# titanium-47/decision-pretrained-transformer

Measured on NVIDIA B200. Metric: env-steps/sec (bandit rollout collect, H=500 dim=5), higher is better.
Workload: dtype f32

## Files before the change

decision-pretrained-transformer_b200/csrc/api.cu:

```cuda
#include "common.cuh"

namespace dpt {

static thread_local char g_err[512] = "";

void set_error(const char* fmt, ...) {
  va_list ap;
  va_start(ap, fmt);
  vsnprintf(g_err, sizeof(g_err), fmt, ap);
  va_end(ap);
}

int sm_count() {
  static thread_local int cached_dev = -1, cached = 0;
  int dev = 0;
  if (cudaGetDevice(&dev) != cudaSuccess) return 148;
  if (dev != cached_dev) {
    int n = 0;
    if (cudaDeviceGetAttribute(&n, cudaDevAttrMultiProcessorCount, dev) != cudaSuccess || n <= 0) n = 148;
    cached = n;
    cached_dev = dev;
  }
  return cached;
}

int pick_envs_per_cta(int N, int slots, int min_e, int max_e) {
  if (min_e < 1) min_e = 1;
  if (max_e < min_e) max_e = min_e;
  if (slots < 1) slots = 1;
  int best = -1;
  double best_eff = -1.0;
  for (int e = max_e; e >= min_e; --e) {
    const long grid = ((long)N + e - 1) / e;
    const long waves = (grid + slots - 1) / slots;
    if (waves < 3 && e > min_e) continue;
    const double eff = (double)grid / (double)(waves * slots);
    if (eff > best_eff + 1e-9) best_eff = eff, best = e;
  }
  return best < 0 ? min_e : best;
}

}

extern "C" int dpt_version(void) { return DPT_ABI_VERSION; }

extern "C" const char* dpt_last_error(void) { return dpt::g_err; }

extern "C" int dpt_device_info(int* sm_count, int* cc_major, int* cc_minor) {
  int dev = 0;
  DPT_CUDA(cudaGetDevice(&dev));
  int n = 0, maj = 0, min = 0;
  DPT_CUDA(cudaDeviceGetAttribute(&n, cudaDevAttrMultiProcessorCount, dev));
  DPT_CUDA(cudaDeviceGetAttribute(&maj, cudaDevAttrComputeCapabilityMajor, dev));
  DPT_CUDA(cudaDeviceGetAttribute(&min, cudaDevAttrComputeCapabilityMinor, dev));
  if (sm_count) *sm_count = n;
  if (cc_major) *cc_major = maj;
  if (cc_minor) *cc_minor = min;
  return DPT_OK;
}
```

decision-pretrained-transformer_b200/csrc/bandit_rollin.cu:

```cuda
#include <string.h>

#include <unordered_map>

#include "common.cuh"
#include "philox.cuh"

namespace dpt {

constexpr int RB_THREADS = 256;
constexpr int RB_WARPS = RB_THREADS / 32;
constexpr int RB_MAX_ENVS = 32;
constexpr int RB_MAX_D = 32;

enum { MODE_PHILOX = 0, MODE_PHILOX_DUMP = 1, MODE_INJECT = 2 };

struct RollinParams {
  const float* means;
  float var;
  int rtype;
  Key key;
  uint64_t env_id0;
  int N, H, d, envs_per_cta;
  float *ctx_s, *ctx_a, *ctx_ns, *ctx_r;
  uint8_t* acts_u8;
  double* stats;
  dpt_bandit_inject_t in;
  dpt_bandit_dump_t out;
};

__constant__ double c_cov_grid[11] = {0.0, .1, .2, .3, .4, .5, .6, .7, .8, .9, 1.0};

template <int MODE>
struct Thr {
  using type = uint32_t;
};
template <>
struct Thr<MODE_INJECT> {
  using type = double;
};

template <int MODE, int DMAX>
__device__ __forceinline__ void rollin_setup_env(const RollinParams& p, int env, int D, float* s_means,
                                                 typename Thr<MODE>::type* s_thr) {
  const uint64_t gid = p.env_id0 + (uint64_t)env;
  for (int j = 0; j < D; ++j) s_means[j] = p.means[(size_t)env * D + j];
  if (MODE == MODE_INJECT && p.in.actions != nullptr) return;
  int cov_idx, ridx;
  double probs[DMAX];
  if (MODE == MODE_INJECT) {
    cov_idx = p.in.cov_idx[env];
    ridx = p.in.rand_idx[env];
#pragma unroll
    for (int j = 0; j < DMAX; ++j)
      if (j < D) probs[j] = p.in.dir_probs[(size_t)env * D + j];
  } else {
    const uint4 w = philox_words(p.key, gid, 0, STREAM_ROLLIN_SETUP);
    cov_idx = (int)bounded(w.x, 11);
    ridx = (int)bounded(w.y, (uint32_t)D);
    double sum = 0.0;
#pragma unroll
    for (int b = 0; b < (DMAX + 3) / 4; ++b) {
      if (4 * b < D) {
        const uint4 g = philox_words(p.key, gid, 1 + b, STREAM_ROLLIN_SETUP);
#pragma unroll
        for (int i = 0; i < 4; ++i) {
          const int j = 4 * b + i;
          if (j < DMAX && j < D) {
            probs[j] = (double)(-__logf(u32_open0(word_of(g, i))));
            sum += probs[j];
          }
        }
      }
    }
// ... 29 lines not shown
      }
    }
  }
}

__device__ __forceinline__ void reduce_stats(const RollinParams& p, float sr, float sr2, float nopt) {
  double* stats = p.stats;
  __shared__ float s_part[3][RB_WARPS];
  const int lane = threadIdx.x & 31, warp = threadIdx.x >> 5;
#pragma unroll
  for (int o = 16; o > 0; o >>= 1) {
    sr += __shfl_xor_sync(0xffffffffu, sr, o);
    sr2 += __shfl_xor_sync(0xffffffffu, sr2, o);
    nopt += __shfl_xor_sync(0xffffffffu, nopt, o);
  }
  if (lane == 0) s_part[0][warp] = sr, s_part[1][warp] = sr2, s_part[2][warp] = nopt;
  __syncthreads();
  if (threadIdx.x < 3) {
    double acc = 0.0;
    for (int w = 0; w < RB_WARPS; ++w) acc += (double)s_part[threadIdx.x][w];
    atomicAdd(stats + threadIdx.x, acc);
  }
}

struct PeerPublish {
  double* dst[DPT_MAX_PEERS];
  int n;
};
__global__ void peer_publish_kernel(const double* __restrict__ stats, const PeerPublish pp) {
  const int r = threadIdx.x / 3, t = threadIdx.x - 3 * r;
  if (r < pp.n) asm volatile("st.global.relaxed.sys.f64 [%0], %1;" ::"l"(pp.dst[r] + t), "d"(stats[t]) : "memory");
}

__device__ __forceinline__ float2 add2(float2 a, float2 b) {
  float2 r;
  asm("add.rn.f32x2 %0, %1, %2;" : "=l"(reinterpret_cast<uint64_t&>(r)) : "l"(reinterpret_cast<uint64_t&>(a)), "l"(reinterpret_cast<uint64_t&>(b)));
  return r;
}
__device__ __forceinline__ float2 fma2(float2 a, float2 b, float2 c) {
  float2 r;
  asm("fma.rn.f32x2 %0, %1, %2, %3;"
      : "=l"(reinterpret_cast<uint64_t&>(r))
      : "l"(reinterpret_cast<uint64_t&>(a)), "l"(reinterpret_cast<uint64_t&>(b)), "l"(reinterpret_cast<uint64_t&>(c)));
  return r;
}

__device__ __forceinline__ int argmax_first(const float* m, int D) {
  int best = 0;
  for (int j = 1; j < D; ++j)
    if (m[j] > m[best]) best = j;
  return best;
}

template <int D, int MODE, int RT>
__global__ void __launch_bounds__(RB_THREADS) bandit_rollin_fast(const RollinParams p) {
  using thr_t = typename Thr<MODE>::type;
  __shared__ float s_means[RB_MAX_ENVS][D];
  __shared__ thr_t s_thr[RB_MAX_ENVS][D];
  __shared__ uint32_t s_optmask[RB_MAX_ENVS];
  const int tid = threadIdx.x, lane = tid & 31, warp = tid >> 5;
  const int env0 = blockIdx.x * p.envs_per_cta;
  const int ne = min(p.envs_per_cta, p.N - env0);
  const int H = p.H;

  if (warp == 0) {
    if (lane < ne) {
      rollin_setup_env<MODE, D>(p, env0 + lane, D, s_means[lane], s_thr[lane]);
      const int oa = argmax_first(s_means[lane], D);
      s_optmask[lane] = (1u << oa) | (1u << (D + oa));
    }
  } else {
    const size_t b = (size_t)env0 * H, e = (size_t)(env0 + ne) * H;
    fill_range(p.ctx_s, b, e, 1.0f, tid - 32, RB_THREADS - 32);
    fill_range(p.ctx_ns, b, e, 1.0f, tid - 32, RB_THREADS - 32);
  }
  __syncthreads();

  const int chunks = (H + 63) >> 6;
  const bool inj_actions = (MODE == MODE_INJECT) && p.in.actions != nullptr;
  float2 st_r = make_float2(0.f, 0.f), st_r2 = make_float2(0.f, 0.f);
  int st_opt = 0;
  const int de = RB_WARPS / chunks, dc = RB_WARPS - de * chunks;
  int e = warp / chunks, c = warp - e * chunks;
  for (; e < ne; e += de, c += dc) {
    if (c >= chunks) {
      c -= chunks, ++e;
      if (e >= ne) break;
    }
    const int env = env0 + e;
    const int h0 = c * 64 + 2 * lane;
    const size_t row = (size_t)env * H + h0;
    int a0 = 0, a1 = 0;
    float z0 = 0.f, z1 = 0.f;
    if (MODE != MODE_INJECT) {
      const uint4 w = philox_words(p.key, p.env_id0 + (uint64_t)env, (uint32_t)(c * 32 + lane), STREAM_ROLLIN_STEP);
      const uint32_t k0 = w.x >> 1, k1 = w.y >> 1;
#pragma unroll
      for (int j = 0; j < D - 1; ++j) {
        const uint32_t t = s_thr[e][j];
        a0 += (k0 >= t);
        a1 += (k1 >= t);
      }
      if (RT == DPT_REWARD_GAUSSIAN)
        box_muller(w.z, w.w, z0, z1);
      else
        z0 = u24(w.z), z1 = u24(w.w);
      if (MODE == MODE_PHILOX_DUMP && h0 < H) {
        if (p.out.u) {
          p.out.u[row] = (double)k0 * 4.656612873077392578125e-10;
          p.out.u[row + 1] = (double)k1 * 4.656612873077392578125e-10;
        }
        if (p.out.z) p.out.z[row] = z0, p.out.z[row + 1] = z1;
        if (p.out.actions) p.out.actions[row] = a0, p.out.actions[row + 1] = a1;
      }
    } else if (h0 < H) {
      if (inj_actions) {
        a0 = p.in.actions[row];
        a1 = p.in.actions[row + 1];
      } else {
        const double u0 = p.in.u[row], u1 = p.in.u[row + 1];
#pragma unroll
        for (int j = 0; j < D - 1; ++j) {
          const double t = s_thr[e][j];
          a0 += (t <= u0);
          a1 += (t <= u1);
        }
      }
      z0 = p.in.z[row];
      z1 = p.in.z[row + 1];
    }
    {
      const float m0 = s_means[e][a0], m1 = s_means[e][a1];
      const bool gauss = RT == DPT_REWARD_GAUSSIAN;
      const float r0 = gauss ? fmaf(p.var, z0, m0) : (z0 < m0 ? 1.f : 0.f);
      const float r1 = gauss ? fmaf(p.var, z1, m1) : (z1 < m1 ? 1.f : 0.f);
      st_stream_if(h0 < H, reinterpret_cast<float2*>(p.ctx_r + row), make_float2(r0, r1));
      if (p.stats && h0 < H) {
        const float2 rr = make_float2(r0, r1);
        st_r = add2(st_r, rr);
        st_r2 = fma2(rr, rr, st_r2);
      }
    }
    const uint32_t m = (1u << a0) | (1u << (D + a1));
    if (p.stats && h0 < H) st_opt += __popc(m & s_optmask[e]);
    float4* abase = reinterpret_cast<float4*>(p.ctx_a + ((size_t)env * H + (size_t)c * 64) * D);
    const int n_valid4 = (min(64, H - c * 64) * D) >> 2;
#pragma unroll
    for (int it = 0; it < (16 * D + 31) / 32; ++it) {
      const int q = it * 32 + lane;
      const int e0 = 4 * q;
      const int l0 = e0 / (2 * D);
      const int off = e0 - l0 * (2 * D);
      const uint32_t mlo = __shfl_sync(0xffffffffu, m, l0 & 31);
      const uint32_t mhi = __shfl_sync(0xffffffffu, m, (l0 + 1) & 31);
      const uint32_t bits = (uint32_t)(((((uint64_t)mhi) << (2 * D)) | mlo) >> off);
      const float4 v = make_float4((bits & 1u) ? 1.f : 0.f, (bits & 2u) ? 1.f : 0.f, (bits & 4u) ? 1.f : 0.f,
                                   (bits & 8u) ? 1.f : 0.f);
      st_stream_if(q < n_valid4, abase + q, v);
    }
  }
  if (p.stats) reduce_stats(p, st_r.x + st_r.y, st_r2.x + st_r2.y, (float)st_opt);
}

template <int MODE>
__global__ void __launch_bounds__(RB_THREADS) bandit_rollin_generic(const RollinParams p) {
  using thr_t = typename Thr<MODE>::type;
  __shared__ float s_means[RB_MAX_ENVS][RB_MAX_D];
  __shared__ thr_t s_thr[RB_MAX_ENVS][RB_MAX_D];
  __shared__ int s_opt[RB_MAX_ENVS];
  const int tid = threadIdx.x, lane = tid & 31, warp = tid >> 5;
  const int env0 = blockIdx.x * p.envs_per_cta;
  const int ne = min(p.envs_per_cta, p.N - env0);
  const int H = p.H, D = p.d;

  if (tid < ne) {
    rollin_setup_env<MODE, RB_MAX_D>(p, env0 + tid, D, s_means[tid], s_thr[tid]);
    s_opt[tid] = argmax_first(s_means[tid], D);
  }
  if (!p.acts_u8) {
    for (size_t i = (size_t)env0 * H + tid; i < (size_t)(env0 + ne) * H; i += RB_THREADS) {
      st_stream(p.ctx_s + i, 1.0f);
      st_stream(p.ctx_ns + i, 1.0f);
    }
  }
  __syncthreads();

  const int chunks = (H + 31) >> 5;
  const bool inj_actions = (MODE == MODE_INJECT) && p.in.actions != nullptr;
  float st_r = 0.f, st_r2 = 0.f, st_opt = 0.f;
  for (int task = warp; task < ne * chunks; task += RB_WARPS) {
    const int e = task / chunks, c = task - e * chunks;
    const int env = env0 + e;
    const int h = c * 32 + lane;
    const size_t row = (size_t)env * H + h;
    int a = 0;
    float z = 0.f;
    if (MODE != MODE_INJECT) {
      const uint4 w = philox_words(p.key, p.env_id0 + (uint64_t)env, (uint32_t)(h >> 1), STREAM_ROLLIN_STEP);
      const uint32_t k = ((h & 1) ? w.y : w.x) >> 1;
      for (int j = 0; j < D - 1; ++j) a += (k >= s_thr[e][j]);
      if (p.rtype == DPT_REWARD_GAUSSIAN) {
        float z0, z1;
        box_muller(w.z, w.w, z0, z1);
        z = (h & 1) ? z1 : z0;
      } else {
        z = u24((h & 1) ? w.w : w.z);
      }
      if (MODE == MODE_PHILOX_DUMP && h < H) {
        if (p.out.u) p.out.u[row] = (double)k * 4.656612873077392578125e-10;
        if (p.out.z) p.out.z[row] = z;
        if (p.out.actions) p.out.actions[row] = a;
      }
    } else if (h < H) {
      if (inj_actions) {
        a = p.in.actions[row];
      } else {
        const double u = p.in.u[row];
        for (int j = 0; j < D - 1; ++j) a += (s_thr[e][j] <= u);
      }
      z = p.in.z[row];
    }
    if (h < H) {
      const float ma = s_means[e][a];
      const float r = p.rtype == DPT_REWARD_GAUSSIAN ? fmaf(p.var, z, ma) : (z < ma ? 1.f : 0.f);
      st_stream(p.ctx_r + row, r);
      if (p.stats) st_r += r, st_r2 = fmaf(r, r, st_r2), st_opt += (float)(a == s_opt[e]);
    }
    if (p.acts_u8) {
      if (h < H) p.acts_u8[row] = (uint8_t)a;
      continue;
    }
    const int nvalid = min(32, H - c * 32) * D;
    float* abase = p.ctx_a + ((size_t)env * H + (size_t)c * 32) * D;
    for (int it = 0; it < D; ++it) {
      const int i = it * 32 + lane;
      const int s = i / D;
      const int as = __shfl_sync(0xffffffffu, a, s & 31);
      if (i < nvalid) st_stream(abase + i, (i - s * D) == as ? 1.f : 0.f);
    }
  }
  if (p.stats) reduce_stats(p, st_r, st_r2, st_opt);
}

template <typename K>
static int resident_ctas(K kern) {
  static thread_local std::unordered_map<const void*, int> cache;
  const void* key = reinterpret_cast<const void*>(kern);
  auto it = cache.find(key);
  if (it != cache.end()) return it->second;
  int n = 0;
  if (cudaOccupancyMaxActiveBlocksPerMultiprocessor(&n, kern, RB_THREADS, 0) != cudaSuccess || n < 1) n = 4;
  cache[key] = n;
  return n;
}

template <int MODE>
static void launch_mode(RollinParams p, bool fast, cudaStream_t st) {
  auto go = [&](auto kern) {
    const int per_sm = resident_ctas(kern);
    p.envs_per_cta = pick_envs_per_cta(p.N, sm_count() * per_sm, 1, RB_MAX_ENVS);
    const int grid = (p.N + p.envs_per_cta - 1) / p.envs_per_cta;
    kern<<<grid, RB_THREADS, 0, st>>>(p);
  };
  if (fast) {
    switch (p.d) {
#define DPT_CASE(DD)                                                   \
  case DD:                                                             \
    if (p.rtype == DPT_REWARD_GAUSSIAN)                                \
      go(bandit_rollin_fast<DD, MODE, DPT_REWARD_GAUSSIAN>);           \
    else                                                               \
      go(bandit_rollin_fast<DD, MODE, DPT_REWARD_BERNOULLI>);          \
    return;
      DPT_CASE(2)
      DPT_CASE(3)
      DPT_CASE(4)
      DPT_CASE(5)
      DPT_CASE(6)
      DPT_CASE(8)
      DPT_CASE(10)
      DPT_CASE(16)
#undef DPT_CASE
      default:
        break;
    }
  }
  go(bandit_rollin_generic<MODE>);
}

}

using namespace dpt;

static int bandit_rollin_impl(const float* means, float var, int reward_type, uint64_t seed, uint64_t env_id0, int N, int H, int d,
                              float* ctx_states, float* ctx_actions, float* ctx_next_states, float* ctx_rewards,
                              double* return_stats, const dpt_bandit_inject_t* inject, const dpt_bandit_dump_t* dump,
                              double* const* peer_dst, int n_peers, unsigned int* done_counter, void* stream,
                              uint8_t* acts_u8 = nullptr) {
  DPT_CHECK_ARG(N >= 0 && H >= 0, "dpt_bandit_rollin: N=%d H=%d must be >= 0", N, H);
  DPT_CHECK_ARG(reward_type == DPT_REWARD_GAUSSIAN || reward_type == DPT_REWARD_BERNOULLI,
                "dpt_bandit_rollin: unknown reward_type %d (0 uniform/gaussian, 1 bernoulli)", reward_type);
  DPT_CHECK_ARG(d >= 1 && d <= RB_MAX_D, "dpt_bandit_rollin: d=%d outside [1,%d]", d, RB_MAX_D);
  if (N == 0 || H == 0) return DPT_OK;
  DPT_CHECK_ARG(means && ctx_rewards && (acts_u8 || (ctx_states && ctx_actions && ctx_next_states)),
                "dpt_bandit_rollin: null means/context pointer");
  RollinParams p{};
  p.acts_u8 = acts_u8;
  p.means = means;
  p.var = var;
  p.rtype = reward_type;
  p.key = Key{(uint32_t)seed, (uint32_t)(seed >> 32)};
  p.env_id0 = env_id0;
  p.N = N, p.H = H, p.d = d;
  p.ctx_s = ctx_states, p.ctx_a = ctx_actions, p.ctx_ns = ctx_next_states, p.ctx_r = ctx_rewards;
  p.stats = return_stats;
  if (n_peers > 0)
    DPT_CHECK_ARG(n_peers <= DPT_MAX_PEERS && peer_dst && return_stats,
                  "dpt_bandit_rollin_p2p: needs return_stats and 1..%d peer pointers", DPT_MAX_PEERS);
  int mode = MODE_PHILOX;
  if (inject) {
    DPT_CHECK_ARG(!dump, "dpt_bandit_rollin: inject and dump are mutually exclusive");
    DPT_CHECK_ARG(inject->z, "dpt_bandit_rollin: inject->z is required");
    DPT_CHECK_ARG(inject->actions || (inject->cov_idx && inject->dir_probs && inject->rand_idx && inject->u),
                  "dpt_bandit_rollin: inject needs actions or (cov_idx, dir_probs, rand_idx, u)");
    p.in = *inject;
    mode = MODE_INJECT;
  } else if (dump) {
    p.out = *dump;
    mode = MODE_PHILOX_DUMP;
  }
  const bool fast = !acts_u8 && (H % 4 == 0) && 2 * d <= 32 && aligned16(ctx_states) && aligned16(ctx_actions) &&
                    aligned16(ctx_next_states) && aligned16(ctx_rewards);
  cudaStream_t st = (cudaStream_t)stream;
  if (mode == MODE_PHILOX)
    launch_mode<MODE_PHILOX>(p, fast, st);
  else if (mode == MODE_PHILOX_DUMP)
    launch_mode<MODE_PHILOX_DUMP>(p, fast, st);
  else
    launch_mode<MODE_INJECT>(p, fast, st);
  DPT_LAUNCH_CHECK();
  if (n_peers > 0) {
    PeerPublish pp{};
    for (int r = 0; r < n_peers; ++r) pp.dst[r] = peer_dst[r];
    pp.n = n_peers;
    peer_publish_kernel<<<1, 3 * DPT_MAX_PEERS <= 32 ? 32 : 3 * DPT_MAX_PEERS, 0, st>>>(return_stats, pp);
    DPT_LAUNCH_CHECK();
  }
  (void)done_counter;
  return DPT_OK;
}

extern "C" int dpt_bandit_rollin(const float* means, float var, int reward_type, uint64_t seed, uint64_t env_id0, int N, int H, int d,
                                 float* ctx_states, float* ctx_actions, float* ctx_next_states, float* ctx_rewards,
                                 double* return_stats, const dpt_bandit_inject_t* inject,
                                 const dpt_bandit_dump_t* dump, void* stream) {
  return bandit_rollin_impl(means, var, reward_type, seed, env_id0, N, H, d, ctx_states, ctx_actions, ctx_next_states,
                            ctx_rewards, return_stats, inject, dump, nullptr, 0, nullptr, stream);
}

namespace dpt {
int bandit_rollin_compact(const float* means, float var, uint64_t seed, uint64_t env_id0, int N, int H, int d, uint8_t* acts_u8,
                          float* ctx_rewards, void* stream) {
  return bandit_rollin_impl(means, var, DPT_REWARD_GAUSSIAN, seed, env_id0, N, H, d, nullptr, nullptr, nullptr, ctx_rewards,
                            nullptr, nullptr, nullptr, nullptr, 0, nullptr, stream, acts_u8);
// ... 52 lines not shown
```

decision-pretrained-transformer_b200/csrc/common.cuh:

```cuda
#pragma once
#include <cuda_runtime.h>
#include <stdint.h>
#include <stdio.h>
#include <stdarg.h>

#include "../../include/dpt_b200.h"

#if defined(__CUDA_ARCH__) && (__CUDA_ARCH__ < 1000)
#error "libdpt_b200 is written for sm_100a (B200) only"
#endif

namespace dpt {

void set_error(const char* fmt, ...);
int sm_count();
int bandit_rollin_compact(const float* means, float var, uint64_t seed, uint64_t env_id0, int N, int H, int d, uint8_t* acts_u8,
                          float* ctx_rewards, void* stream);
int pick_envs_per_cta(int N, int slots, int min_e, int max_e);

#define DPT_CHECK_ARG(cond, ...)                \
  do {                                          \
    if (!(cond)) {                              \
      dpt::set_error(__VA_ARGS__);              \
      return DPT_ERR_INVALID_ARG;               \
    }                                           \
  } while (0)

#define DPT_CUDA(call)                                                                  \
  do {                                                                                  \
    cudaError_t _e = (call);                                                            \
    if (_e != cudaSuccess) {                                                            \
      dpt::set_error("%s failed: %s (%s:%d)", #call, cudaGetErrorString(_e), __FILE__, __LINE__); \
      return DPT_ERR_CUDA;                                                              \
    }                                                                                   \
  } while (0)

#define DPT_LAUNCH_CHECK()                                                              \
  do {                                                                                  \
    cudaError_t _e = cudaGetLastError();                                                \
    if (_e != cudaSuccess) {                                                            \
      dpt::set_error("kernel launch failed: %s (%s:%d)", cudaGetErrorString(_e), __FILE__, __LINE__); \
      return DPT_ERR_CUDA;                                                              \
    }                                                                                   \
  } while (0)

static inline bool aligned16(const void* p) { return (reinterpret_cast<uintptr_t>(p) & 15) == 0; }

#ifdef __CUDACC__
__device__ __forceinline__ void st_stream(float4* p, float4 v) {
  asm volatile("st.global.L1::no_allocate.v4.f32 [%0], {%1, %2, %3, %4};" ::"l"(p), "f"(v.x), "f"(v.y), "f"(v.z),
               "f"(v.w)
               : "memory");
}
__device__ __forceinline__ void st_stream_if(bool pred, float4* p, float4 v) {
  asm volatile(
      "{\n\t.reg .pred p;\n\tsetp.ne.b32 p, %5, 0;\n\t@p st.global.L1::no_allocate.v4.f32 [%0], {%1, %2, %3, %4};\n\t}"
      ::"l"(p), "f"(v.x), "f"(v.y), "f"(v.z), "f"(v.w), "r"((int)pred)
      : "memory");
}
__device__ __forceinline__ void st_stream_if(bool pred, float2* p, float2 v) {
  asm volatile("{\n\t.reg .pred p;\n\tsetp.ne.b32 p, %3, 0;\n\t@p st.global.L1::no_allocate.v2.f32 [%0], {%1, %2};\n\t}" ::"l"(p),
               "f"(v.x), "f"(v.y), "r"((int)pred)
               : "memory");
}
__device__ __forceinline__ void st_stream(float2* p, float2 v) {
  asm volatile("st.global.L1::no_allocate.v2.f32 [%0], {%1, %2};" ::"l"(p), "f"(v.x), "f"(v.y) : "memory");
}
__device__ __forceinline__ void st_stream(float* p, float v) {
  asm volatile("st.global.L1::no_allocate.f32 [%0], %1;" ::"l"(p), "f"(v) : "memory");
}

__device__ __forceinline__ void fill_range(float* base, size_t begin, size_t end, float v, int tid, int nthreads) {
  const size_t mis = (reinterpret_cast<uintptr_t>(base + begin) >> 2) & 3;
  size_t b4 = begin + ((4 - mis) & 3);
  if (b4 > end) b4 = end;
  const size_t e4 = b4 + ((end - b4) & ~size_t(3));
  if (tid < (int)(b4 - begin)) st_stream(base + begin + tid, v);
  if (tid < (int)(end - e4)) st_stream(base + e4 + tid, v);
  const float4 v4 = make_float4(v, v, v, v);
  float4* p = reinterpret_cast<float4*>(base + b4);
  const size_t n4 = (e4 - b4) >> 2;
  for (size_t i = tid; i < n4; i += nthreads) st_stream(p + i, v4);
}
#endif

}
```

decision-pretrained-transformer_b200/csrc/online_loop.cu:

```cuda
#include <cstdlib>

#include <atomic>

#include "online_loop.cuh"

namespace dpt {

__host__ __device__ inline size_t ol_arms_offset(int nwarps, int dmax) {
  return (sizeof(WarpTile) * nwarps + sizeof(float) * 32 * nwarps * dmax + 7) & ~size_t(7);
}

template <int DMAX, int KIND, bool IO>
__global__ void __launch_bounds__(OL_THREADS) online_loop_kernel(const OnlineParams p) {
  extern __shared__ __align__(16) unsigned char smem_raw[];
  __shared__ float4 s_nib[16];
  const int nthreads = blockDim.x, nwarps = nthreads >> 5;
  WarpTile* tiles = reinterpret_cast<WarpTile*>(smem_raw);
  float* s_means_all = reinterpret_cast<float*>(smem_raw + sizeof(WarpTile) * nwarps);
  double* s_arms = reinterpret_cast<double*>(smem_raw + ol_arms_offset(nwarps, DMAX));
  const int tid = threadIdx.x, lane = tid & 31, warp = tid >> 5;
  WarpTile& tile = tiles[warp];
  float(*s_means)[DMAX] = reinterpret_cast<float(*)[DMAX]>(s_means_all) + warp * 32;
  const int env0w = (blockIdx.x * nwarps + warp) * 32;
  if (tid < 16) s_nib[tid] = make_float4((tid & 1) ? 1.f : 0.f, (tid & 2) ? 1.f : 0.f, (tid & 4) ? 1.f : 0.f, (tid & 8) ? 1.f : 0.f);
  const int env = env0w + lane;
  const bool live = env < p.N;
  const int N = p.N, H = p.H, d = p.d;
  const uint64_t gid = p.env_id0 + (uint64_t)env;
  const bool materialise = p.ctx_a != nullptr;

  if (KIND == K_LINUCB || KIND == K_LINUCB2) {
    for (int i = tid; i < d * p.lin_d; i += nthreads) s_arms[i] = p.arms[i];
  }
  float m[DMAX];
  float mmax = -INFINITY;
  int opt = 0;
#pragma unroll
  for (int j = 0; j < DMAX; ++j) {
    m[j] = (live && j < d) ? p.means[(size_t)env * d + j] : -INFINITY;
    if (m[j] > mmax) mmax = m[j], opt = j;
    s_means[lane][j] = m[j];
  }
  __syncthreads();


  if (p.ctx_s) {
    const int nl = min(32, N - env0w);
    if (nl > 0) {
      fill_range(p.ctx_s, (size_t)env0w * H, (size_t)(env0w + nl) * H, 1.0f, lane, 32);
      fill_range(p.ctx_ns, (size_t)env0w * H, (size_t)(env0w + nl) * H, 1.0f, lane, 32);
    }
  }

  ArmState<DMAX> st;
#pragma unroll
  for (int j = 0; j < DMAX; ++j) {
    st.sum[j] = 0.0, st.cnt[j] = 0;
    st.aux0[j] = (KIND == K_THOMPSON) ? p.p1 : 0.0;
    st.aux1[j] = (KIND == K_THOMPSON) ? sqrt(p.p2) : p.p0;
  }
  double S[KIND == K_LINUCB ? OL_MAX_LD * OL_MAX_LD : 1], bv[KIND == K_LINUCB ? OL_MAX_LD : 1];
  double s00 = 1.0, s01 = 0.0, s11 = 1.0, b0 = 0.0, b1 = 0.0;
  if (KIND == K_LINUCB) {
    for (int i = 0; i < p.lin_d; ++i) {
      bv[i] = 0.0;
      for (int j = 0; j < p.lin_d; ++j) S[i * p.lin_d + j] = (i == j) ? 1.0 : 0.0;
    }
  }
  const double sigma2 = p.p0 * p.p0;
  double creg = 0.0;
  const int nb_ctrl = (d + 3) >> 2;

  float zc[KIND == K_THOMPSON ? DMAX : 1];
  auto gen_ctrl = [&](int h, float* out) {
    if (IO && p.in.ctrl_z) {
#pragma unroll
      for (int j = 0; j < DMAX; ++j) out[j] = (live && j < d) ? p.in.ctrl_z[((size_t)h * N + env) * d + j] : 0.f;
// ... 423 lines not shown
```

decision-pretrained-transformer_b200/csrc/online_loop_ws.cu:

```cuda
#include <stdlib.h>

#include "online_loop.cuh"

namespace dpt {

#ifndef DPT_WS_WT5
#define DPT_WS_WT5 32
#endif
#ifndef DPT_WS_WT10
#define DPT_WS_WT10 16
#endif
#ifndef DPT_WS_STAGGER
#define DPT_WS_STAGGER 0
#endif
#ifndef DPT_WS_FILL_TILE
#define DPT_WS_FILL_TILE 0
#endif
#ifndef DPT_WS_SKIP
#define DPT_WS_SKIP 0
#endif
#ifndef DPT_WS_NCONS
#define DPT_WS_NCONS 4
#endif
template <int DMAX>
// ... 400 lines not shown
  static __device__ __forceinline__ void controller_split(const OnlineParams& p, const SplitArgs& sa, Cons& cs, const double* s_arms,
                                                          const double* __restrict__ tab0, const double* __restrict__ tab1, int env, bool live,
                                                          int lane) {
    const int H = p.H, d = p.d;
    const uint64_t gid = p.env_id0 + (uint64_t)env;
    const double sigma2tc0 = p.p0 * p.p0 * p.p1;
    float mmax = -INFINITY;
    int opt = 0;
    State S;
#pragma unroll
    for (int j = 0; j < DMAX; ++j) {
      const bool real = j < d;
      const float mj = (live && real) ? p.means[(size_t)env * d + j] : -INFINITY;
      if (mj > mmax) mmax = mj, opt = j;
      cs.means[lane][j] = mj;
      if (STATS) cs.sum[j][lane] = 0.0, cs.cnt[j][lane] = 0;
      if (KIND == K_EMP) S.st0[j] = real ? 0.0 : -INFINITY;
      if (KIND == K_UCB) S.st0[j] = real ? 0.0 + p.p0 : -INFINITY;
      if (KIND == K_THOMPSON) S.st0[j] = real ? p.p1 : -INFINITY, S.st1[j] = real ? sqrt(p.p2) : 0.0;
    }
    S.untried = (1u << d) - 1u;
    S.s00 = 1.0, S.s01 = 0.0, S.s11 = 1.0, S.b0 = 0.0, S.b1 = 0.0;
    __syncwarp();
    float* cmp = p.cum_means + env;
    SplitLane sl{};
    sl.arms4 = sa.arms4 ? sa.arms4 + env : nullptr, sl.creg_out = sa.creg ? sa.creg + env : nullptr, sl.mmax = (double)mmax;
    if (sa.creg && live) sa.creg[(size_t)((H + 127) >> 7) * p.N + env] = (double)mmax;
    if (sa.fill) {
      const int env0 = env - lane;
      const long long run = (long long)min(32, p.N - env0) * H - 4 * lane;
      sl.fill_n = run > 0 ? (int)((run + 127) >> 7) : 0;
      sl.fill_p = reinterpret_cast<float4*>(p.ctx_s + (size_t)env0 * H) + lane;
      sl.fill_off = reinterpret_cast<char*>(p.ctx_ns) - reinterpret_cast<char*>(p.ctx_s);
    }
    const int nq = H >> 2, rem = H & 3;
#pragma unroll 1
    for (int q = 0; q < nq; ++q) quad<true>(p, cs, S, s_arms, tab0, tab1, 4 * q, 4, q, opt, env, live, gid, cmp, sigma2tc0, false, lane, sl);
    if (rem) quad<false>(p, cs, S, s_arms, tab0, tab1, 4 * nq, rem, nq, opt, env, live, gid, cmp, sigma2tc0, false, lane, sl);
  }
};

template <int DMAX, int KIND>
constexpr int ws_min_blocks() { return (DMAX > 5 && KIND == K_THOMPSON) ? 4 : 6; }

template <int DMAX, int KIND, bool IO>
__global__ void __launch_bounds__(WS_NCONS * 32, ws_min_blocks<DMAX, KIND>()) online_loop_ws_kernel(const OnlineParams p, const double* __restrict__ tab) {
  using K = WsKernel<DMAX, KIND, IO>;
  using Cons = typename K::Cons;
  extern __shared__ __align__(16) unsigned char smem_raw[];
  __shared__ float4 s_nib[16];
  Cons* cons = reinterpret_cast<Cons*>(smem_raw);
  double* s_arms = reinterpret_cast<double*>(smem_raw + sizeof(Cons) * WS_NCONS);
  const int tid = threadIdx.x, lane = tid & 31, warp = tid >> 5;
  if (tid < 16) s_nib[tid] = make_float4((tid & 1) ? 1.f : 0.f, (tid & 2) ? 1.f : 0.f, (tid & 4) ? 1.f : 0.f, (tid & 8) ? 1.f : 0.f);
  if (KIND == K_LINUCB2)
    for (int j = tid; j < p.d; j += blockDim.x) lin_arm_row(s_arms + LIN_AW * j, p.arms[2 * j], p.arms[2 * j + 1]);
  __syncthreads();
  const int env = (blockIdx.x * WS_NCONS + warp) * 32 + lane;
  if (env - lane < p.N)
    K::controller(p, cons[warp], s_arms, s_nib, tab, tab + (p.H + 1), env, env < p.N, lane);
}

template <int DMAX, int KIND>
constexpr int ctrl_min_blocks() { return (DMAX > 5 && KIND == K_THOMPSON) ? 4 : 6; }
#ifndef DPT_CTRL_MINB
#define DPT_CTRL_MINB (ctrl_min_blocks<DMAX, KIND>())
#endif
#ifndef DPT_EX_MINB
#define DPT_EX_MINB (REG ? (D > 5 ? 5 : 6) : 8)
#endif
template <int DMAX, int KIND, bool IO>
__global__ void __launch_bounds__(WS_NCONS * 32, DPT_CTRL_MINB) online_ctrl_kernel(const OnlineParams p, const double* __restrict__ tab,
                                                                                                   const SplitArgs sa) {
  using K = WsKernel<DMAX, KIND, IO, true>;
  using Cons = typename K::Cons;
  DPT_TL(1);
  extern __shared__ __align__(16) unsigned char smem_raw[];
  Cons* cons = reinterpret_cast<Cons*>(smem_raw);
  double* s_arms = reinterpret_cast<double*>(smem_raw + sizeof(Cons) * WS_NCONS);
  const int tid = threadIdx.x, lane = tid & 31, warp = tid >> 5;
  if (KIND == K_LINUCB2) {
    for (int j = tid; j < p.d; j += blockDim.x) lin_arm_row(s_arms + LIN_AW * j, p.arms[2 * j], p.arms[2 * j + 1]);
    __syncthreads();
  }
  const int env = (blockIdx.x * WS_NCONS + warp) * 32 + lane;
  if (env - lane < p.N)
    K::controller_split(p, sa, cons[warp], s_arms, tab, tab + (p.H + 1), env, env < p.N, lane);
}

constexpr int EX_WARPS = 4;
constexpr int EX_Q = 32;
constexpr int EX_TASKS = 32;

template <int D, bool INJ, bool REG>
__global__ void __launch_bounds__(EX_WARPS * 32, DPT_EX_MINB) online_expand_kernel(const OnlineParams p, const uint32_t* __restrict__ arms4,
                                                                                   const double* __restrict__ creg_in, int nqt, int ngy) {
  DPT_TL(10);
  __shared__ float4 s_nib[16];
  __shared__ uint32_t s_arm[EX_WARPS][EX_Q][33];
  if (threadIdx.x < 16) {
    const int t = threadIdx.x;
    s_nib[t] = make_float4((t & 1) ? 1.f : 0.f, (t & 2) ? 1.f : 0.f, (t & 4) ? 1.f : 0.f, (t & 8) ? 1.f : 0.f);
  }
  __syncthreads();
  const int lane = threadIdx.x & 31, warp = threadIdx.x >> 5;
  const int N = p.N, H = p.H;
  const int W = blockIdx.x * EX_WARPS + warp;
  const int bx = W / ngy, by = W - bx * ngy;
  const int env0 = bx * EX_TASKS, ne = min(EX_TASKS, N - env0);
  const int q0 = by * EX_Q, nq = min(EX_Q, nqt - q0);
  if (ne <= 0) return;
  const int q = q0 + lane;
  const bool qv = lane < nq;
#pragma unroll 8
  for (int k = 0; k < nq; ++k) s_arm[warp][k][lane] = lane < ne ? __ldcs(arms4 + (size_t)(q0 + k) * N + env0 + lane) : 0u;
  __syncwarp();
  const float* msrc = p.means + (size_t)env0 * D + (lane < D ? lane : 0);
  const double* csrc = creg_in + (size_t)by * N + env0;
  float m_n = __ldg(msrc);
  const double* xsrc = creg_in + (size_t)ngy * N + env0;
  double c_n = REG ? __ldg(csrc) : 0.0, x_n = REG ? __ldg(xsrc) : 0.0;
  double s1[4] = {0.0, 0.0, 0.0, 0.0}, s2[4] = {0.0, 0.0, 0.0, 0.0}, c2[4] = {0.0, 0.0, 0.0, 0.0};
  for (int e = 0; e < ne; ++e) {
    const int env = env0 + e;
    const uint32_t aw = qv ? s_arm[warp][lane][e] : 0u;
    const float m = m_n;
    const double carry = c_n, mmax = x_n;
    if (e + 1 < ne) {
      m_n = __ldg(msrc + (e + 1) * D);
      if (REG) c_n = __ldg(csrc + e + 1), x_n = __ldg(xsrc + e + 1);
    }
    float zz[4];
    if (INJ) {
#pragma unroll
      for (int t = 0; t < 4; ++t) zz[t] = qv ? p.in.reward_z[(size_t)(4 * q + t) * N + env] : 0.f;
    } else {
      reward_noise4(p.key, p.env_id0 + (uint64_t)env, (uint32_t)q, p.rtype, zz);
    }
    float rr[4], ma[4];
    uint64_t bq = 0ull;
#pragma unroll
    for (int u = 0; u < 4; ++u) {
      const int a = qv ? (aw >> (8 * u)) & 255 : 0;
      ma[u] = __shfl_sync(0xffffffffu, m, a);
      rr[u] = (float)reward_f64(ma[u], zz[u], p.var, p.rtype);
      bq |= (uint64_t)(1u << a) << (u * D);
    }
    const size_t row = (size_t)env * H + 4 * (size_t)q0;
    st_stream_if(qv, reinterpret_cast<float4*>(p.ctx_r + row) + lane, make_float4(rr[0], rr[1], rr[2], rr[3]));
    double reg[4], sc = 0.0;
    if (REG) {
#pragma unroll
      for (int u = 0; u < 4; ++u) reg[u] = qv ? mmax - (double)ma[u] : 0.0;
      sc = ((reg[0] + reg[1]) + reg[2]) + reg[3];
    }
    auto scan_round = [&](int o) {
      const double v = __shfl_up_sync(0xffffffffu, sc, o);
      if (lane >= o) sc += v;
    };
    float4* abase = reinterpret_cast<float4*>(p.ctx_a + row * D);
    const uint32_t blo = (uint32_t)bq, bhi = (uint32_t)(bq >> 32);
    const int nvalid = nq * D;
#pragma unroll
    for (int it = 0; it < D; ++it) {
      const int g = it * 32 + lane;
      const int src = g / D, f = g - src * D;
      uint32_t w = __shfl_sync(0xffffffffu, blo, src);
      if (4 * D > 32) {
        const uint32_t wh = __shfl_sync(0xffffffffu, bhi, src);
        w = (uint32_t)((((uint64_t)wh << 32) | w) >> (4 * f));
      } else {
        w >>= 4 * f;
      }
      st_stream_if(g < nvalid, abase + g, s_nib[w & 15u]);
      if (REG && it < 5) scan_round(1 << it);
    }
    if (REG) {
#pragma unroll
      for (int it = D; it < 5; ++it) scan_round(1 << it);
      double cr = carry + (sc - (((reg[0] + reg[1]) + reg[2]) + reg[3]));
#pragma unroll
      for (int u = 0; u < 4; ++u) {
        cr += reg[u];
        s1[u] += reg[u], s2[u] = fma(reg[u], reg[u], s2[u]), c2[u] = fma(cr, cr, c2[u]);
      }
    }
  }
  if (REG && qv) {
    double* acc = p.regret + 3 * ((size_t)(bx & (p.regret_reps - 1)) * H + 4 * (size_t)q);
#pragma unroll
    for (int u = 0; u < 4; ++u) atomicAdd(acc + 3 * u, s1[u]), atomicAdd(acc + 3 * u + 1, s2[u]), atomicAdd(acc + 3 * u + 2, c2[u]);
  }
}

__global__ void __launch_bounds__(EX_WARPS * 32) online_expand_generic_kernel(const OnlineParams p, const uint32_t* __restrict__ arms4, int q_lo,
                                                                              int q_hi) {
  DPT_TL(10);
  const int lane = threadIdx.x & 31, warp = threadIdx.x >> 5;
  const int N = p.N, H = p.H, d = p.d;
  const int env = blockIdx.x * EX_WARPS + warp;
  if (env >= N) return;
  const bool inj = p.in.reward_z != nullptr;
  for (int q = q_lo + lane; q < q_hi; q += 32) {
    const uint32_t aw = arms4[(size_t)q * N + env];
    float zz[4];
    if (inj) {
#pragma unroll
      for (int t = 0; t < 4; ++t) zz[t] = (4 * q + t < H) ? p.in.reward_z[(size_t)(4 * q + t) * N + env] : 0.f;
    } else {
      reward_noise4(p.key, p.env_id0 + (uint64_t)env, (uint32_t)q, p.rtype, zz);
    }
#pragma unroll
    for (int u = 0; u < 4; ++u) {
      const int h = 4 * q + u;
      if (h >= H) break;
      const int a = (aw >> (8 * u)) & 255;
      const size_t row = (size_t)env * H + h;
      st_stream(p.ctx_r + row, (float)reward_f64(p.means[(size_t)env * d + a], zz[u], p.var, p.rtype));
      for (int j = 0; j < d; ++j) st_stream(p.ctx_a + row * d + j, j == a ? 1.f : 0.f);
    }
  }
}

__global__ void __launch_bounds__(256) ones_fill_kernel(float* __restrict__ a, float* __restrict__ b, size_t n) {
  DPT_TL(0);
  const size_t per = ((n + gridDim.x - 1) / gridDim.x + 3) & ~size_t(3);
  const size_t lo = min(n, per * blockIdx.x), hi = min(n, lo + per);
  fill_range(a, lo, hi, 1.0f, threadIdx.x, 256);
  fill_range(b, lo, hi, 1.0f, threadIdx.x, 256);
// ... 297 lines not shown
```

decision-pretrained-transformer_b200/csrc/philox.cuh:

```cuda
#pragma once
#include <stdint.h>

namespace dpt {

enum : uint32_t {
  STREAM_TASK = 0,
  STREAM_ROLLIN_SETUP = 1,
  STREAM_ROLLIN_STEP = 2,
  STREAM_DARKROOM_STEP = 3,
  STREAM_DARKROOM_QUERY = 4,
  STREAM_ENV_REWARD = 5,
  STREAM_CTRL = 6,
};

struct Key {
  uint32_t k0, k1;
};

__device__ __forceinline__ uint4 philox4x32_10(uint32_t c0, uint32_t c1, uint32_t c2, uint32_t c3, Key key) {
  uint32_t k0 = key.k0, k1 = key.k1;
#pragma unroll
  for (int r = 0; r < 10; ++r) {
    uint32_t hi0 = __umulhi(0xD2511F53u, c0), lo0 = 0xD2511F53u * c0;
    uint32_t hi1 = __umulhi(0xCD9E8D57u, c2), lo1 = 0xCD9E8D57u * c2;
    c0 = hi1 ^ c1 ^ k0;
    c1 = lo1;
    c2 = hi0 ^ c3 ^ k1;
    c3 = lo0;
    k0 += 0x9E3779B9u;
    k1 += 0xBB67AE85u;
  }
  return make_uint4(c0, c1, c2, c3);
}

__device__ __forceinline__ uint4 philox_words(Key key, uint64_t env, uint32_t index, uint32_t stream) {
  return philox4x32_10(index, (uint32_t)env, (uint32_t)(env >> 32), stream, key);
}

__device__ __forceinline__ uint32_t word_of(uint4 w, int i) {
  return i == 0 ? w.x : i == 1 ? w.y : i == 2 ? w.z : w.w;
}

__device__ __forceinline__ uint32_t bounded(uint32_t w, uint32_t n) { return __umulhi(w, n); }

__device__ __forceinline__ float u24(uint32_t w) { return (float)(w >> 8) * 5.9604644775390625e-08f; }

__device__ __forceinline__ float u32_open0(uint32_t w) {
  return fmaf((float)w, 2.3283064365386963e-10f, 1.1641532182693481e-10f);
}

__device__ __forceinline__ float fast_lg2(float x) {
  float y;
  asm("lg2.approx.ftz.f32 %0, %1;" : "=f"(y) : "f"(x));
  return y;
}
__device__ __forceinline__ float fast_sqrt(float x) {
  float y;
  asm("sqrt.approx.ftz.f32 %0, %1;" : "=f"(y) : "f"(x));
  return y;
}
__device__ __forceinline__ void box_muller(uint32_t a, uint32_t b, float& z0, float& z1) {
  float r = fast_sqrt(-1.3862943611198906f * fast_lg2(u32_open0(a)));
  float s, c;
  __sincosf((float)b * 1.4629180792671596e-09f , &s, &c);
  z0 = r * c;
  z1 = r * s;
}

}
```

Measured before the change: 198.1 billion.

## Process four steps per lane in bandit rollin with shared one-hot store and precomputed Philox keys

New measurement: 212.3 billion (median of 6 runs). 1.07x the previous value.

```diff
diff --git a/decision-pretrained-transformer_b200/csrc/api.cu b/decision-pretrained-transformer_b200/csrc/api.cu
--- a/decision-pretrained-transformer_b200/csrc/api.cu
+++ b/decision-pretrained-transformer_b200/csrc/api.cu
@@ -24,19 +24,21 @@
   return cached;
 }
 
-int pick_envs_per_cta(int N, int slots, int min_e, int max_e) {
+int pick_envs_per_cta(int N, int slots, int min_e, int max_e, int step) {
   if (min_e < 1) min_e = 1;
   if (max_e < min_e) max_e = min_e;
   if (slots < 1) slots = 1;
   int best = -1;
   double best_eff = -1.0;
   for (int e = max_e; e >= min_e; --e) {
+    if (step > 1 && e % step) continue;
     const long grid = ((long)N + e - 1) / e;
     const long waves = (grid + slots - 1) / slots;
     if (waves < 3 && e > min_e) continue;
     const double eff = (double)grid / (double)(waves * slots);
     if (eff > best_eff + 1e-9) best_eff = eff, best = e;
   }
+  if (best < 0 && step > 1) return pick_envs_per_cta(N, slots, min_e, max_e, 1);
   return best < 0 ? min_e : best;
 }
 
diff --git a/decision-pretrained-transformer_b200/csrc/bandit_rollin.cu b/decision-pretrained-transformer_b200/csrc/bandit_rollin.cu
--- a/decision-pretrained-transformer_b200/csrc/bandit_rollin.cu
+++ b/decision-pretrained-transformer_b200/csrc/bandit_rollin.cu
@@ -1,5 +1,6 @@
 #include <string.h>
 
+#include <type_traits>
 #include <unordered_map>
 
 #include "common.cuh"
@@ -19,6 +20,7 @@
   float var;
   int rtype;
   Key key;
+  RoundKeys rk;
   uint64_t env_id0;
   int N, H, d, envs_per_cta;
   float *ctx_s, *ctx_a, *ctx_ns, *ctx_r;
@@ -154,22 +156,28 @@
   return best;
 }
 
+#ifndef DPT_RB_MINB
+#define DPT_RB_MINB (D <= 5 ? 5 : D <= 10 ? 4 : 2)
+#endif
 template <int D, int MODE, int RT>
-__global__ void __launch_bounds__(RB_THREADS) bandit_rollin_fast(const RollinParams p) {
+__global__ void __launch_bounds__(RB_THREADS, DPT_RB_MINB) bandit_rollin_fast(const RollinParams p) {
   using thr_t = typename Thr<MODE>::type;
+  using qbits_t = typename std::conditional<(4 * D > 32), uint64_t, uint32_t>::type;
+  __shared__ float4 s_nib[16];
   __shared__ float s_means[RB_MAX_ENVS][D];
   __shared__ thr_t s_thr[RB_MAX_ENVS][D];
-  __shared__ uint32_t s_optmask[RB_MAX_ENVS];
+  __shared__ qbits_t s_optmask[RB_MAX_ENVS];
   const int tid = threadIdx.x, lane = tid & 31, warp = tid >> 5;
   const int env0 = blockIdx.x * p.envs_per_cta;
   const int ne = min(p.envs_per_cta, p.N - env0);
   const int H = p.H;
 
   if (warp == 0) {
+    onehot_nib_init(s_nib, lane);
     if (lane < ne) {
       rollin_setup_env<MODE, D>(p, env0 + lane, D, s_means[lane], s_thr[lane]);
-      const int oa = argmax_first(s_means[lane], D);
-      s_optmask[lane] = (1u << oa) | (1u << (D + oa));
+      const qbits_t o = (qbits_t)1 << argmax_first(s_means[lane], D);
+      s_optmask[lane] = o | (o << D) | (o << (2 * D)) | (o << (3 * D));
     }
   } else {
     const size_t b = (size_t)env0 * H, e = (size_t)(env0 + ne) * H;
@@ -178,7 +186,7 @@
   }
   __syncthreads();
 
-  const int chunks = (H + 63) >> 6;
+  const int chunks = (H + 127) >> 7;
   const bool inj_actions = (MODE == MODE_INJECT) && p.in.actions != nullptr;
   float2 st_r = make_float2(0.f, 0.f), st_r2 = make_float2(0.f, 0.f);
   int st_opt = 0;
@@ -190,76 +198,69 @@
       if (e >= ne) break;
     }
     const int env = env0 + e;
-    const int h0 = c * 64 + 2 * lane;
+    const int h0 = c * 128 + 4 * lane;
+    const bool valid = h0 < H;
     const size_t row = (size_t)env * H + h0;
-    int a0 = 0, a1 = 0;
-    float z0 = 0.f, z1 = 0.f;
+    int a[4] = {0, 0, 0, 0};
+    float z[4] = {0.f, 0.f, 0.f, 0.f};
     if (MODE != MODE_INJECT) {
-      const uint4 w = philox_words(p.key, p.env_id0 + (uint64_t)env, (uint32_t)(c * 32 + lane), STREAM_ROLLIN_STEP);
-      const uint32_t k0 = w.x >> 1, k1 = w.y >> 1;
+      const uint64_t gid = p.env_id0 + (uint64_t)env;
+      const uint4 w0 = philox_words(p.rk, gid, (uint32_t)(h0 >> 1), STREAM_ROLLIN_STEP);
+      const uint4 w1 = philox_words(p.rk, gid, (uint32_t)(h0 >> 1) + 1u, STREAM_ROLLIN_STEP);
+      const uint32_t k[4] = {w0.x >> 1, w0.y >> 1, w1.x >> 1, w1.y >> 1};
 #pragma unroll
       for (int j = 0; j < D - 1; ++j) {
         const uint32_t t = s_thr[e][j];
-        a0 += (k0 >= t);
-        a1 += (k1 >= t);
-      }
-      if (RT == DPT_REWARD_GAUSSIAN)
-        box_muller(w.z, w.w, z0, z1);
-      else
-        z0 = u24(w.z), z1 = u24(w.w);
-      if (MODE == MODE_PHILOX_DUMP && h0 < H) {
-        if (p.out.u) {
-          p.out.u[row] = (double)k0 * 4.656612873077392578125e-10;
-          p.out.u[row + 1] = (double)k1 * 4.656612873077392578125e-10;
+#pragma unroll
+        for (int u = 0; u < 4; ++u) a[u] -= (int)((k[u] - t) >> 31);
+      }
+#pragma unroll
+      for (int u = 0; u < 4; ++u) a[u] += D - 1;
+      if (RT == DPT_REWARD_GAUSSIAN) {
+        box_muller(w0.z, w0.w, z[0], z[1]);
+        box_muller(w1.z, w1.w, z[2], z[3]);
+      } else {
+        z[0] = u24(w0.z), z[1] = u24(w0.w), z[2] = u24(w1.z), z[3] = u24(w1.w);
+      }
+      if (MODE == MODE_PHILOX_DUMP && valid) {
+#pragma unroll
+        for (int u = 0; u < 4; ++u) {
+          if (p.out.u) p.out.u[row + u] = (double)k[u] * 4.656612873077392578125e-10;
+          if (p.out.z) p.out.z[row + u] = z[u];
+          if (p.out.actions) p.out.actions[row + u] = a[u];
         }
-        if (p.out.z) p.out.z[row] = z0, p.out.z[row + 1] = z1;
-        if (p.out.actions) p.out.actions[row] = a0, p.out.actions[row + 1] = a1;
-      }
-    } else if (h0 < H) {
-      if (inj_actions) {
-        a0 = p.in.actions[row];
-        a1 = p.in.actions[row + 1];
-      } else {
-        const double u0 = p.in.u[row], u1 = p.in.u[row + 1];
-#pragma unroll
-        for (int j = 0; j < D - 1; ++j) {
-          const double t = s_thr[e][j];
-          a0 += (t <= u0);
-          a1 += (t <= u1);
+      }
+    } else if (valid) {
+#pragma unroll
+      for (int u = 0; u < 4; ++u) {
+        if (inj_actions) {
+          a[u] = p.in.actions[row + u];
+        } else {
+          const double uu = p.in.u[row + u];
+#pragma unroll
+          for (int j = 0; j < D - 1; ++j) a[u] += (s_thr[e][j] <= uu);
         }
-      }
-      z0 = p.in.z[row];
-      z1 = p.in.z[row + 1];
-    }
-    {
-      const float m0 = s_means[e][a0], m1 = s_means[e][a1];
-      const bool gauss = RT == DPT_REWARD_GAUSSIAN;
-      const float r0 = gauss ? fmaf(p.var, z0, m0) : (z0 < m0 ? 1.f : 0.f);
-      const float r1 = gauss ? fmaf(p.var, z1, m1) : (z1 < m1 ? 1.f : 0.f);
-      st_stream_if(h0 < H, reinterpret_cast<float2*>(p.ctx_r + row), make_float2(r0, r1));
-      if (p.stats && h0 < H) {
-        const float2 rr = make_float2(r0, r1);
-        st_r = add2(st_r, rr);
-        st_r2 = fma2(rr, rr, st_r2);
-      }
-    }
-    const uint32_t m = (1u << a0) | (1u << (D + a1));
-    if (p.stats && h0 < H) st_opt += __popc(m & s_optmask[e]);
-    float4* abase = reinterpret_cast<float4*>(p.ctx_a + ((size_t)env * H + (size_t)c * 64) * D);
-    const int n_valid4 = (min(64, H - c * 64) * D) >> 2;
-#pragma unroll
-    for (int it = 0; it < (16 * D + 31) / 32; ++it) {
-      const int q = it * 32 + lane;
-      const int e0 = 4 * q;
-      const int l0 = e0 / (2 * D);
-      const int off = e0 - l0 * (2 * D);
-      const uint32_t mlo = __shfl_sync(0xffffffffu, m, l0 & 31);
-      const uint32_t mhi = __shfl_sync(0xffffffffu, m, (l0 + 1) & 31);
-      const uint32_t bits = (uint32_t)(((((uint64_t)mhi) << (2 * D)) | mlo) >> off);
-      const float4 v = make_float4((bits & 1u) ? 1.f : 0.f, (bits & 2u) ? 1.f : 0.f, (bits & 4u) ? 1.f : 0.f,
-                                   (bits & 8u) ? 1.f : 0.f);
-      st_stream_if(q < n_valid4, abase + q, v);
-    }
+        z[u] = p.in.z[row + u];
+      }
+    }
+    float r[4];
+    qbits_t bq = 0;
+#pragma unroll
+    for (int u = 0; u < 4; ++u) {
+      const float m = s_means[e][a[u]];
+      r[u] = RT == DPT_REWARD_GAUSSIAN ? fmaf(p.var, z[u], m) : (z[u] < m ? 1.f : 0.f);
+      bq |= ((qbits_t)1 << a[u]) << (u * D);
+    }
+    st_stream_if(valid, reinterpret_cast<float4*>(p.ctx_r + row), make_float4(r[0], r[1], r[2], r[3]));
+    if (p.stats && valid) {
+      const float2 r01 = make_float2(r[0], r[1]), r23 = make_float2(r[2], r[3]);
+      st_r = add2(add2(st_r, r01), r23);
+      st_r2 = fma2(r23, r23, fma2(r01, r01, st_r2));
+      st_opt += 4 * D > 32 ? __popcll((uint64_t)(bq & s_optmask[e])) : __popc((uint32_t)(bq & s_optmask[e]));
+    }
+    const int nq = min(32, (H - c * 128) >> 2);
+    onehot_quad_store<D>(reinterpret_cast<float4*>(p.ctx_a + ((size_t)env * H + (size_t)c * 128) * D), bq, lane, nq * D, s_nib,
+                         [](int) {});
   }
   if (p.stats) reduce_stats(p, st_r.x + st_r.y, st_r2.x + st_r2.y, (float)st_opt);
 }
@@ -358,20 +359,26 @@
 
 template <int MODE>
 static void launch_mode(RollinParams p, bool fast, cudaStream_t st) {
-  auto go = [&](auto kern) {
-    const int per_sm = resident_ctas(kern);
-    p.envs_per_cta = pick_envs_per_cta(p.N, sm_count() * per_sm, 1, RB_MAX_ENVS);
+  auto go = [&](auto kern, int step, int min_e) {
+    const int slots = sm_count() * resident_ctas(kern);
+    p.envs_per_cta = pick_envs_per_cta(p.N, slots, min_e, RB_MAX_ENVS, step);
+    if (min_e > 1 && (p.N + p.envs_per_cta - 1) / p.envs_per_cta < 3 * slots)
+      p.envs_per_cta = pick_envs_per_cta(p.N, slots, 1, RB_MAX_ENVS);
     const int grid = (p.N + p.envs_per_cta - 1) / p.envs_per_cta;
     kern<<<grid, RB_THREADS, 0, st>>>(p);
   };
   if (fast) {
+    const int chunks = (p.H + 127) >> 7;
+    int step = 1;
+    while ((step * chunks) % RB_WARPS) ++step;
+    const int min_e = (4 * RB_WARPS / chunks + step - 1) / step * step;
     switch (p.d) {
 #define DPT_CASE(DD)                                                   \
   case DD:                                                             \
     if (p.rtype == DPT_REWARD_GAUSSIAN)                                \
-      go(bandit_rollin_fast<DD, MODE, DPT_REWARD_GAUSSIAN>);           \
+      go(bandit_rollin_fast<DD, MODE, DPT_REWARD_GAUSSIAN>, step, min_e);  \
     else                                                               \
-      go(bandit_rollin_fast<DD, MODE, DPT_REWARD_BERNOULLI>);          \
+      go(bandit_rollin_fast<DD, MODE, DPT_REWARD_BERNOULLI>, step, min_e); \
     return;
       DPT_CASE(2)
       DPT_CASE(3)
@@ -386,7 +393,7 @@
         break;
     }
   }
-  go(bandit_rollin_generic<MODE>);
+  go(bandit_rollin_generic<MODE>, 1, 1);
 }
 
 }
@@ -411,6 +418,7 @@
   p.var = var;
   p.rtype = reward_type;
   p.key = Key{(uint32_t)seed, (uint32_t)(seed >> 32)};
+  p.rk = round_keys(p.key);
   p.env_id0 = env_id0;
   p.N = N, p.H = H, p.d = d;
   p.ctx_s = ctx_states, p.ctx_a = ctx_actions, p.ctx_ns = ctx_next_states, p.ctx_r = ctx_rewards;
diff --git a/decision-pretrained-transformer_b200/csrc/common.cuh b/decision-pretrained-transformer_b200/csrc/common.cuh
--- a/decision-pretrained-transformer_b200/csrc/common.cuh
+++ b/decision-pretrained-transformer_b200/csrc/common.cuh
@@ -16,7 +16,7 @@
 int sm_count();
 int bandit_rollin_compact(const float* means, float var, uint64_t seed, uint64_t env_id0, int N, int H, int d, uint8_t* acts_u8,
                           float* ctx_rewards, void* stream);
-int pick_envs_per_cta(int N, int slots, int min_e, int max_e);
+int pick_envs_per_cta(int N, int slots, int min_e, int max_e, int step = 1);
 
 #define DPT_CHECK_ARG(cond, ...)                \
   do {                                          \
@@ -82,6 +82,29 @@
   const size_t n4 = (e4 - b4) >> 2;
   for (size_t i = tid; i < n4; i += nthreads) st_stream(p + i, v4);
 }
+
+__device__ __forceinline__ void onehot_nib_init(float4* s_nib, int t) {
+  if (t < 16) s_nib[t] = make_float4((t & 1) ? 1.f : 0.f, (t & 2) ? 1.f : 0.f, (t & 4) ? 1.f : 0.f, (t & 8) ? 1.f : 0.f);
+}
+
+template <int D, typename F>
+__device__ __forceinline__ void onehot_quad_store(float4* abase, uint64_t bq, int lane, int nvalid, const float4* s_nib, F&& per_it) {
+  const uint32_t blo = (uint32_t)bq, bhi = (uint32_t)(bq >> 32);
+#pragma unroll
+  for (int it = 0; it < D; ++it) {
+    const int g = it * 32 + lane;
+    const int src = g / D, f = g - src * D;
+    uint32_t w = __shfl_sync(0xffffffffu, blo, src);
+    if (4 * D > 32) {
+      const uint32_t wh = __shfl_sync(0xffffffffu, bhi, src);
+      w = (uint32_t)((((uint64_t)wh << 32) | w) >> (4 * f));
+    } else {
+      w >>= 4 * f;
+    }
+    st_stream_if(g < nvalid, abase + g, s_nib[w & 15u]);
+    per_it(it);
+  }
+}
 #endif
 
 }
diff --git a/decision-pretrained-transformer_b200/csrc/online_loop.cu b/decision-pretrained-transformer_b200/csrc/online_loop.cu
--- a/decision-pretrained-transformer_b200/csrc/online_loop.cu
+++ b/decision-pretrained-transformer_b200/csrc/online_loop.cu
@@ -22,7 +22,7 @@
   WarpTile& tile = tiles[warp];
   float(*s_means)[DMAX] = reinterpret_cast<float(*)[DMAX]>(s_means_all) + warp * 32;
   const int env0w = (blockIdx.x * nwarps + warp) * 32;
-  if (tid < 16) s_nib[tid] = make_float4((tid & 1) ? 1.f : 0.f, (tid & 2) ? 1.f : 0.f, (tid & 4) ? 1.f : 0.f, (tid & 8) ? 1.f : 0.f);
+  onehot_nib_init(s_nib, tid);
   const int env = env0w + lane;
   const bool live = env < p.N;
   const int N = p.N, H = p.H, d = p.d;
diff --git a/decision-pretrained-transformer_b200/csrc/online_loop_ws.cu b/decision-pretrained-transformer_b200/csrc/online_loop_ws.cu
--- a/decision-pretrained-transformer_b200/csrc/online_loop_ws.cu
+++ b/decision-pretrained-transformer_b200/csrc/online_loop_ws.cu
@@ -476,7 +476,7 @@
   Cons* cons = reinterpret_cast<Cons*>(smem_raw);
   double* s_arms = reinterpret_cast<double*>(smem_raw + sizeof(Cons) * WS_NCONS);
   const int tid = threadIdx.x, lane = tid & 31, warp = tid >> 5;
-  if (tid < 16) s_nib[tid] = make_float4((tid & 1) ? 1.f : 0.f, (tid & 2) ? 1.f : 0.f, (tid & 4) ? 1.f : 0.f, (tid & 8) ? 1.f : 0.f);
+  onehot_nib_init(s_nib, tid);
   if (KIND == K_LINUCB2)
     for (int j = tid; j < p.d; j += blockDim.x) lin_arm_row(s_arms + LIN_AW * j, p.arms[2 * j], p.arms[2 * j + 1]);
   __syncthreads();
@@ -522,10 +522,7 @@
   DPT_TL(10);
   __shared__ float4 s_nib[16];
   __shared__ uint32_t s_arm[EX_WARPS][EX_Q][33];
-  if (threadIdx.x < 16) {
-    const int t = threadIdx.x;
-    s_nib[t] = make_float4((t & 1) ? 1.f : 0.f, (t & 2) ? 1.f : 0.f, (t & 4) ? 1.f : 0.f, (t & 8) ? 1.f : 0.f);
-  }
+  onehot_nib_init(s_nib, threadIdx.x);
   __syncthreads();
   const int lane = threadIdx.x & 31, warp = threadIdx.x >> 5;
   const int N = p.N, H = p.H;
@@ -582,23 +579,9 @@
       const double v = __shfl_up_sync(0xffffffffu, sc, o);
       if (lane >= o) sc += v;
     };
-    float4* abase = reinterpret_cast<float4*>(p.ctx_a + row * D);
-    const uint32_t blo = (uint32_t)bq, bhi = (uint32_t)(bq >> 32);
-    const int nvalid = nq * D;
-#pragma unroll
-    for (int it = 0; it < D; ++it) {
-      const int g = it * 32 + lane;
-      const int src = g / D, f = g - src * D;
-      uint32_t w = __shfl_sync(0xffffffffu, blo, src);
-      if (4 * D > 32) {
-        const uint32_t wh = __shfl_sync(0xffffffffu, bhi, src);
-        w = (uint32_t)((((uint64_t)wh << 32) | w) >> (4 * f));
-      } else {
-        w >>= 4 * f;
-      }
-      st_stream_if(g < nvalid, abase + g, s_nib[w & 15u]);
+    onehot_quad_store<D>(reinterpret_cast<float4*>(p.ctx_a + row * D), bq, lane, nq * D, s_nib, [&](int it) {
       if (REG && it < 5) scan_round(1 << it);
-    }
+    });
     if (REG) {
 #pragma unroll
       for (int it = D; it < 5; ++it) scan_round(1 << it);
diff --git a/decision-pretrained-transformer_b200/csrc/philox.cuh b/decision-pretrained-transformer_b200/csrc/philox.cuh
--- a/decision-pretrained-transformer_b200/csrc/philox.cuh
+++ b/decision-pretrained-transformer_b200/csrc/philox.cuh
@@ -17,24 +17,46 @@
   uint32_t k0, k1;
 };
 
+struct RoundKeys {
+  uint32_t k0[10], k1[10];
+};
+__host__ __device__ inline RoundKeys round_keys(Key key) {
+  RoundKeys rk;
+  for (int r = 0; r < 10; ++r) rk.k0[r] = key.k0 + (uint32_t)r * 0x9E3779B9u, rk.k1[r] = key.k1 + (uint32_t)r * 0xBB67AE85u;
+  return rk;
+}
+
+__device__ __forceinline__ void philox_round(uint32_t& c0, uint32_t& c1, uint32_t& c2, uint32_t& c3, uint32_t k0, uint32_t k1) {
+  const uint32_t hi0 = __umulhi(0xD2511F53u, c0), lo0 = 0xD2511F53u * c0;
+  const uint32_t hi1 = __umulhi(0xCD9E8D57u, c2), lo1 = 0xCD9E8D57u * c2;
+  c0 = hi1 ^ c1 ^ k0;
+  c1 = lo1;
+  c2 = hi0 ^ c3 ^ k1;
+  c3 = lo0;
+}
+
 __device__ __forceinline__ uint4 philox4x32_10(uint32_t c0, uint32_t c1, uint32_t c2, uint32_t c3, Key key) {
   uint32_t k0 = key.k0, k1 = key.k1;
 #pragma unroll
   for (int r = 0; r < 10; ++r) {
-    uint32_t hi0 = __umulhi(0xD2511F53u, c0), lo0 = 0xD2511F53u * c0;
-    uint32_t hi1 = __umulhi(0xCD9E8D57u, c2), lo1 = 0xCD9E8D57u * c2;
-    c0 = hi1 ^ c1 ^ k0;
-    c1 = lo1;
-    c2 = hi0 ^ c3 ^ k1;
-    c3 = lo0;
+    philox_round(c0, c1, c2, c3, k0, k1);
     k0 += 0x9E3779B9u;
     k1 += 0xBB67AE85u;
   }
   return make_uint4(c0, c1, c2, c3);
 }
 
+__device__ __forceinline__ uint4 philox4x32_10(uint32_t c0, uint32_t c1, uint32_t c2, uint32_t c3, const RoundKeys& rk) {
+#pragma unroll
+  for (int r = 0; r < 10; ++r) philox_round(c0, c1, c2, c3, rk.k0[r], rk.k1[r]);
+  return make_uint4(c0, c1, c2, c3);
+}
+
 __device__ __forceinline__ uint4 philox_words(Key key, uint64_t env, uint32_t index, uint32_t stream) {
   return philox4x32_10(index, (uint32_t)env, (uint32_t)(env >> 32), stream, key);
+}
+__device__ __forceinline__ uint4 philox_words(const RoundKeys& rk, uint64_t env, uint32_t index, uint32_t stream) {
+  return philox4x32_10(index, (uint32_t)env, (uint32_t)(env >> 32), stream, rk);
 }
 
 __device__ __forceinline__ uint32_t word_of(uint4 w, int i) {
```
